# biod/sambamba

Measured on NVIDIA H100. Metric: bam_gb_per_s_depth_base, higher is better.
Workload: dtype u32

## Files before the change

include/bdepth.h:

```cpp
#ifndef BDEPTH_H
#define BDEPTH_H

#include <stddef.h>
#include <stdint.h>

#ifdef __cplusplus
extern "C" {
#endif

typedef struct bdepth bdepth_t;

typedef enum {
    BDEPTH_OK = 0,
    BDEPTH_ERR_IO = -1,
    BDEPTH_ERR_FORMAT = -2,
    BDEPTH_ERR_UNSORTED = -3,
    BDEPTH_ERR_NOINDEX = -4,
    BDEPTH_ERR_CUDA = -5,
    BDEPTH_ERR_NCCL = -6,
    BDEPTH_ERR_ARG = -7,
    BDEPTH_ERR_CALLBACK = -8
} bdepth_status;

typedef struct { uint32_t ref_id, start, end; } bdepth_region;
// ... 34 lines not shown
    uint64_t covered_positions;
    uint64_t long_reads;
    uint64_t chain_fixups;
    uint32_t gpu_launches;
    uint32_t n_batches;
    float ms_h2d, ms_inflate, ms_scan, ms_coverage, ms_reduce, ms_d2h, ms_total_device;
    double host_wall_ms;
    float ms_span_device;
    float ms_exchange;
    uint64_t own_lo, own_hi;
    uint64_t halo_bytes_sent;
    uint64_t mate_pairs;
    uint64_t mate_pair_columns;
    uint64_t mate_groups;
    float ms_mates;
} bdepth_stats;

int  bdepth_device_count(void);
int  bdepth_open(const char* bam_path, int device, bdepth_t** out);
int  bdepth_open_lazy(const char* bam_path, int device, bdepth_t** out);
int  bdepth_open_memory(const void* bam, size_t bam_len, const void* bai, size_t bai_len, int device, bdepth_t** out);
int  bdepth_add_input(bdepth_t* h, const char* bam_path);
void bdepth_close(bdepth_t* h);
const char* bdepth_last_error(const bdepth_t* h);

int         bdepth_n_ref(const bdepth_t* h);
const char* bdepth_ref_name(const bdepth_t* h, int i);
uint32_t    bdepth_ref_length(const bdepth_t* h, int i);
const char* bdepth_header_text(const bdepth_t* h, size_t* len);
int         bdepth_is_coordinate_sorted(const bdepth_t* h);
// ... 54 lines not shown
```

sambamba_b200/_lib.py:

```python
import ctypes as C
import os
import numpy as np

_HERE = os.path.dirname(os.path.abspath(__file__))


def lib_path():
    return os.path.join(_HERE, "_build", "libbdepth.so")


class BDepthError(RuntimeError):
    def __init__(self, code, msg):
        super().__init__(f"bdepth error {code}: {msg}")
        self.code = code
        self.msg = msg


class Region(C.Structure):
    _fields_ = [("ref_id", C.c_uint32), ("start", C.c_uint32), ("end", C.c_uint32)]


class Tile(C.Structure):
    _fields_ = [("ref_id", C.c_int32), ("start", C.c_uint32), ("len", C.c_uint32), ("stride", C.c_uint32),
                ("counts", C.POINTER(C.c_uint32)), ("n_samples", C.c_uint32), ("sample_stride", C.c_uint32)]


class RegionStat(C.Structure):
    _fields_ = [("ref_id", C.c_int32), ("start", C.c_uint32), ("end", C.c_uint32), ("n_reads", C.c_uint32),
                ("n_bases", C.c_uint32), ("cov_ge", C.POINTER(C.c_uint32)), ("sample_id", C.c_int32)]


class Stats(C.Structure):
    _fields_ = [(n, C.c_uint64) for n in ("file_bytes", "n_blocks", "cdata_bytes", "inflated_bytes", "n_records",
                                          "n_records_pass", "n_cigar_ops", "seq_bytes", "positions",
                                          "covered_positions", "long_reads", "chain_fixups")] + \
               [("gpu_launches", C.c_uint32), ("n_batches", C.c_uint32)] + \
               [(n, C.c_float) for n in ("ms_h2d", "ms_inflate", "ms_scan", "ms_coverage", "ms_reduce", "ms_d2h",
                                         "ms_total_device")] + [("host_wall_ms", C.c_double), ("ms_span_device", C.c_float), ("ms_exchange", C.c_float),
                                                                 ("own_lo", C.c_uint64), ("own_hi", C.c_uint64), ("halo_bytes_sent", C.c_uint64),
                                                                 ("mate_pairs", C.c_uint64), ("mate_pair_columns", C.c_uint64), ("mate_groups", C.c_uint64), ("ms_mates", C.c_float)]

    def as_dict(self):
        return {n: getattr(self, n) for n, _ in self._fields_}


FLAGSTAT_FIELDS = ("total", "secondary", "supplementary", "duplicates", "mapped", "paired", "read1", "read2", "proper_pair", "both_mapped",
                   "singletons", "mate_diff_chr", "mate_diff_chr_mapq5")


class FlagStat(C.Structure):
    _fields_ = [(n, C.c_uint64 * 2) for n in FLAGSTAT_FIELDS]

    def as_dict(self):
        return {n: (getattr(self, n)[0], getattr(self, n)[1]) for n in FLAGSTAT_FIELDS}

# ... 359 lines not shown
```

sambamba_b200/csrc/bdepth.cu:

```cuda
#include "launch.cuh"
#include <dlfcn.h>
#include <fcntl.h>
#include <stdarg.h>
#include <stdio.h>
#include <stdlib.h>
#include <sys/mman.h>
#include <sys/stat.h>
#include <unistd.h>
#include <algorithm>
#include <chrono>
#include <map>
#include <string>
#include <vector>

#include "../../include/bdepth.h"
#include "host_bam.hpp"
#include "kernels.cuh"
#include "mates.cuh"
#include "host_filter.hpp"

using namespace bdk;

namespace {

// ... 23 lines not shown
        e = cudaHostGetDevicePointer((void**)&dp, hp, 0);
        if (e == cudaSuccess) cap = n + n / 4;
        used = 0;
        return e;
    }
    uint8_t* take(size_t n) { size_t a = (used + 15) & ~size_t(15); if (a + n > cap) return nullptr; used = a + n; return hp + a; }
    uint8_t* dev(const void* host) const { return dp + ((const uint8_t*)host - hp); }
    void release() { if (hp) cudaFreeHost(hp); hp = nullptr; dp = nullptr; cap = used = 0; }
};
__global__ void k_copy_words(uint32_t* __restrict__ dst, const uint32_t* __restrict__ src, size_t n) {
    for (size_t i = (size_t)blockIdx.x * blockDim.x + threadIdx.x; i < n; i += (size_t)gridDim.x * blockDim.x) dst[i] = src[i];
}

#ifdef BDEPTH_EMULATE_SHIM
constexpr unsigned COUNT_GRID = 4;
#else
constexpr unsigned COUNT_GRID = 2048;
#endif
constexpr size_t CARRY_MAX = 64ull << 20;
constexpr size_t EMIT_CHUNK = 4ull << 20;
constexpr uint32_t SHARD_EXTRA_BLOCKS = 8;
constexpr uint32_t MATE_ZONE_BLOCKS = 64;

enum RunMode { RUN_FULL = 0, RUN_INFLATE_ONLY = 1, RUN_SCAN_ONLY = 2, RUN_INDEX = 3, RUN_FLAGSTAT = 4, RUN_VIEW_COUNT = 5 };
constexpr int RC_RETRY_WINDOW = 1;

struct NcclUid { char b[128]; };
typedef void* NcclComm;
struct NcclApi {
    bool ok = false; std::string err;
    int (*GetUniqueId)(NcclUid*) = nullptr;
    int (*CommInitRank)(NcclComm*, int, NcclUid, int) = nullptr;
// ... 56 lines not shown
    bool k1lz_v12 = false;
    bool k1lz_flat = false;
    int k1h_variant = -1;
    bool k1_onephase = false;
    bool k3_pre = false;
    bool k3_tile = true;
    bool has_fprog = false; FilterProg fprog; DevBuf fprog_d;
    DevBuf m_hash, m_flag, m_flt, m_ctl;
    uint32_t S = 1;
    DevBuf rg_ids, rg_offs, rg_samp;
    DevBuf text[2], text_tiles, text_offs, text_zero, text_samp, present;
    int coll_pending = 0;
    bool want_presence = false;
    uint64_t batch_u = 6ull << 30;
    uint64_t chunk_blocks = 13 * 32 * 16;
    bool shard_ready = false;
    size_t blk_lo = 0, blk_hi = 0; int64_t entry0 = 0; uint64_t limit_abs_u = 0;
    uint64_t zone_lin_lo = UINT64_MAX;
    uint64_t own_lo_abs_u = 0;
    bool sparse_ok = true;
    bool sparse_on = false;
    std::vector<HostBlock> vblocks; std::vector<int32_t> seg_entry ; std::vector<uint32_t> seg_limit ;
    DevBuf anchors_idx, anchors_val, chunk_limit;
    cudaStream_t s_main = nullptr, s_copy = nullptr, s_d2h = nullptr;
    cudaEvent_t ev[32] = {};
    DevBuf comp2[2];
    cudaStream_t s_k1[16] = {};
    std::vector<cudaEvent_t> chunk_ev[2], k1_ev;
    std::vector<size_t> chunk_end[2];
    bool staged = false; uint64_t staged_file_off = 0;
    DevBuf tok, lits, aux, segi, littab;
    DevBuf comp, descs, status, ubuf, chunk_start, entry, exitb, count, slot_base, slots, rec_base, walk_list;
    DevBuf soa_start, soa_span, soa_meta, soa_off, soa_ncl, soa_lseq, long_list, tile_first, tile_lo, counts, ref_len_d, ref_lin0_d, scan_stats, ref_has, ref_has_all, flt_d, lead_list, misc;
    uint64_t cnt_base = 0, win_len = 0;
    void* pinned = nullptr; size_t pinned_cap = 0;
    HostScratch hs;
    std::vector<uint32_t> ref_has_host;
    struct SegSet { bool on = false; uint32_t n = 0; bool has_min = false, has_u = false; uint64_t ext_max = 0; DevBuf s, e, pmax, id, reads, minstart, bases_reads, mbases, ustart, da, dac, db, dthr, dbases, dcov, dscr; } seg;
    struct IndexSet { DevBuf lin, lin_len, lin_base, lin_cap, n_mapped, n_unmapped, carry, ctl, runs, excs; std::vector<uint32_t> base, cap; std::vector<IndexRun> h_runs; std::vector<IndexExc> h_excs; uint64_t n_lin = 0; } ix;
    std::vector<uint8_t> built_bai;
    DevBuf fs; uint64_t fs_host[FS_WORDS + 1] = {};
    ViewSel vsel{}; DevBuf vc, vc_reg, vc_prog; uint64_t vc_host[2] = {};
    std::vector<bdepth*> extra;
    bool accum = false;
    bool force_window = false;
    bdepth_stats st{}; std::string err;
// ... 13 lines not shown
    if (n <= h->pinned_cap) return 0;
    if (h->pinned) cudaFreeHost(h->pinned);
    h->hs.release();
    h->pinned = nullptr; h->pinned_cap = 0;
    CK(cudaMallocHost(&h->pinned, n));
    h->pinned_cap = n;
    return 0;
}

int init_device(bdepth* h) {
    int n = 0; cudaError_t e = cudaGetDeviceCount(&n);
    if (e != cudaSuccess || n <= 0) return fail(h, BDEPTH_ERR_CUDA, "no CUDA device available (%s); libbdepth has no CPU fallback", cudaGetErrorString(e));
    if (h->device < 0 || h->device >= n) return fail(h, BDEPTH_ERR_ARG, "device %d out of range (%d devices)", h->device, n);
    CK(cudaSetDevice(h->device));
    CK(cudaDeviceGetAttribute(&h->n_sm, cudaDevAttrMultiProcessorCount, h->device));
    if (!h->s_main) { CK(cudaStreamCreateWithFlags(&h->s_main, cudaStreamNonBlocking)); CK(cudaStreamCreateWithFlags(&h->s_copy, cudaStreamNonBlocking)); CK(cudaStreamCreateWithFlags(&h->s_d2h, cudaStreamNonBlocking)); for (auto& ks : h->s_k1) CK(cudaStreamCreateWithFlags(&ks, cudaStreamNonBlocking)); for (auto& e2 : h->ev) CK(cudaEventCreate(&e2)); }
    CK(cudaFuncSetAttribute(k1_inflate, cudaFuncAttributeMaxDynamicSharedMemorySize, K1_SMEM));
    CK(cudaFuncSetAttribute(k1_fallback, cudaFuncAttributeMaxDynamicSharedMemorySize, K1_SMEM));
    CK(cudaFuncSetAttribute(k1_huff<false, 4>, cudaFuncAttributePreferredSharedMemoryCarveout, cudaSharedmemCarveoutMaxShared)); CK(cudaFuncSetAttribute(k1_huff<false, 6>, cudaFuncAttributePreferredSharedMemoryCarveout, cudaSharedmemCarveoutMaxShared));
    CK(cudaFuncSetAttribute(k1_huff<true, 5>, cudaFuncAttributePreferredSharedMemoryCarveout, cudaSharedmemCarveoutMaxShared)); CK(cudaFuncSetAttribute(k1_huff<true, 4>, cudaFuncAttributePreferredSharedMemoryCarveout, cudaSharedmemCarveoutMaxShared));
    { const char* e = getenv("BDEPTH_K1H_VARIANT"); h->k1h_variant = e ? atoi(e) : -1; }
    { const char* e = getenv("BDEPTH_K3"); h->k3_tile = !(e && !strcmp(e, "gather")); }
    CK(cudaFuncSetAttribute(k3_tile<false>, cudaFuncAttributeMaxDynamicSharedMemorySize, (int)K3T_SMEM)); CK(cudaFuncSetAttribute(k3_tile<true>, cudaFuncAttributeMaxDynamicSharedMemorySize, (int)K3T_SMEM));
    { const char* e = getenv("BDEPTH_K1LZ"); h->k1lz_flat = e && !strcmp(e, "flat"); h->k1lz_v12 = e && !strcmp(e, "v12"); }
    { const char* e = getenv("BDEPTH_K1_ONEPHASE"); h->k1_onephase = e && atoi(e) == 1; }
    { const char* e = getenv("BDEPTH_K3_PREFETCH"); h->k3_pre = !e || atoi(e) != 0; }
    return 0;
}

int inflate_blocks_to_host(bdepth* h, size_t b0, size_t b1, std::vector<uint8_t>& out) {
    size_t nb = b1 - b0; if (!nb) { out.clear(); return 0; }
// ... 335 lines not shown
__global__ void k_scatter_i64(int64_t* __restrict__ dst, const uint32_t* __restrict__ idx, const int64_t* __restrict__ val, uint32_t n) {
    uint32_t i = blockIdx.x * blockDim.x + threadIdx.x; if (i < n) dst[idx[i]] = val[i];
}

struct RunOut {
    uint8_t* inflate_dst = nullptr; uint64_t inflate_cap = 0; uint64_t inflate_len = 0;
    uint64_t scan_cap = 0; uint64_t scan_n = 0;
    int32_t* ref_id = nullptr; int32_t* pos = nullptr; uint32_t* span = nullptr; uint16_t* flag = nullptr; uint8_t* mapq = nullptr; uint16_t* n_cigar = nullptr; uint64_t* rec_off = nullptr;
};

__global__ void k_fill_u32(uint32_t* p, uint32_t v, uint64_t n) { uint64_t i = (uint64_t)blockIdx.x * blockDim.x + threadIdx.x; if (i < n) p[i] = v; }

int run_pipeline_body(bdepth* h, RunMode mode, RunOut* ro, Emitter* em);
int run_pipeline(bdepth* h, RunMode mode, RunOut* ro, Emitter* em = nullptr) {
    const int rc = run_pipeline_body(h, mode, ro, em);
    if (rc && rc != RC_RETRY_WINDOW) abort_collectives(h);
    return rc;
}
int run_pipeline_body(bdepth* h, RunMode mode, RunOut* ro, Emitter* em) {
    h->coll_pending = 0;
    int rc = init_device(h); if (rc) return rc;
    auto t_host0 = std::chrono::steady_clock::now();
    bdepth_stats& st = h->st; uint32_t launches0 = 0;
    st = bdepth_stats{}; st.gpu_launches = launches0;
    const bool sparse = (mode == RUN_FULL || mode == RUN_VIEW_COUNT) && plan_sparse(h);
    h->coll_pending = (mode == RUN_FULL && h->world > 1 && h->comm) ? (sparse ? 2 : 1) : (mode == RUN_FLAGSTAT && h->world > 1 && h->comm) ? 3 : (mode == RUN_VIEW_COUNT && h->world > 1 && h->comm) ? (sparse ? 2 : 4) : 0;
    if (!sparse) { rc = prepare_shard(h); if (rc) return rc; }
    const bool fix = mode == RUN_FULL && h->fix_mates;
    bool flt_uploaded = false;
    if (fix && h->world > 1 && !h->comm) return fail(h, BDEPTH_ERR_ARG, "fix-mate-overlaps on several ranks needs the boundary exchange (bdepth_set_shard with a NCCL id)");
// ... 172 lines not shown
            const HostBlock& hb = B[b + i];
            uint64_t dev_off = h->staged ? hb.coff - h->staged_file_off : dco[batch_no & 1][i];
            d[i] = BlockDesc{dev_off + hb.cdata_off, hb.uoff - batch_u0, hb.csize, hb.isize, tok_words};
            tok_words += tok_cap_of(hb.isize);
            if (b + i >= new_b) { csum += hb.csize; st.file_bytes += hb.bsize; }
        }
        st.cdata_bytes += csum;
        CK(h->descs.ensure(nb * sizeof(BlockDesc))); CK(h->status.ensure(nb * sizeof(int))); CK(h->ubuf.ensure(CARRY_MAX + ub + 256));
        if (!h->k1_onephase) { CK(h->tok.ensure(tok_words * 4 + 64)); CK(h->lits.ensure(ub + 16 * nb + 64)); CK(h->aux.ensure(nb * sizeof(BlockAux))); CK(h->segi.ensure(nb * MAX_SEG * 4)); CK(h->littab.ensure(nb * (size_t)MAX_SEG * 256)); }
        CK(hs.ensure(nb * (sizeof(BlockDesc) + 192) + 16384)); hs.used = 0;
        UP(h->descs.p, d.data(), nb * sizeof(BlockDesc));
        uint8_t* u0 = h->ubuf.as<uint8_t>() + CARRY_MAX;
        CK(cudaEventRecord(e1, sm));
        struct Sub { size_t s0, s1; int ev_lo, ev_hi; };
        std::vector<Sub> subs;
        auto launch_k1 = [&](cudaStream_t ks, size_t c0, uint32_t n) -> int {
            const BlockDesc* dd = h->descs.as<BlockDesc>() + (c0 - b); int* stp = h->status.as<int>() + (c0 - b);
            if (h->k1_onephase) {
                BD_LAUNCH((n + 32 * K1_WARPS - 1) / (32 * K1_WARPS), 32 * K1_WARPS, K1_SMEM, ks, k1_inflate)(d_comp, dd, n, u0, stp);
                CK(cudaGetLastError()); st.gpu_launches++;
                return 0;
            }
            BlockAux* ax = h->aux.as<BlockAux>() + (c0 - b); uint32_t* sgi = h->segi.as<uint32_t>() + (c0 - b) * MAX_SEG; uint8_t* ltb = h->littab.as<uint8_t>() + (c0 - b) * (size_t)MAX_SEG * 256;
            const unsigned hg = (n + 32 * K1H_WARPS - 1) / (32 * K1H_WARPS); const uint32_t blk0 = (uint32_t)(c0 - b);
#define K1H(LIMS, MINB) BD_LAUNCH(hg, 32 * K1H_WARPS, k1h_smem<LIMS>(), ks, k1_huff<LIMS, MINB>)(d_comp, dd, n, blk0, stp, h->tok.as<uint32_t>(), h->lits.as<uint8_t>(), ax, sgi, ltb)
            const int variant = h->k1h_variant >= 0 ? h->k1h_variant : (n > (uint32_t)h->n_sm * 16u * 32u ? 2 : 0);
            switch (variant) { case 1: K1H(false, 6); break; case 2: K1H(true, 5); break; case 3: K1H(true, 4); break; default: K1H(false, 4); }
#undef K1H
            if (h->k1lz_flat) BD_LAUNCH((n + K1L_WARPS - 1) / K1L_WARPS, 32 * K1L_WARPS, 0, ks, k1_lz_flat)(dd, n, blk0, u0, stp, h->tok.as<uint32_t>(), h->lits.as<uint8_t>(), ax, sgi, ltb);
            else if (h->k1lz_v12) BD_LAUNCH((n + K1L_WARPS - 1) / K1L_WARPS, 32 * K1L_WARPS, 0, ks, k1_lz<false>)(dd, n, blk0, u0, stp, h->tok.as<uint32_t>(), h->lits.as<uint8_t>(), ax, sgi, ltb);
            else BD_LAUNCH((n + K1L_WARPS - 1) / K1L_WARPS, 32 * K1L_WARPS, 0, ks, k1_lz<true>)(dd, n, blk0, u0, stp, h->tok.as<uint32_t>(), h->lits.as<uint8_t>(), ax, sgi, ltb);
            BD_LAUNCH((n + 32 * K1_WARPS - 1) / (32 * K1_WARPS), 32 * K1_WARPS, K1_SMEM, ks, k1_fallback)(d_comp, dd, n, u0, stp);
            CK(cudaGetLastError()); st.gpu_launches += 3;
            return 0;
        };
        if (h->staged) {
            { int rck = launch_k1(sm, b, (uint32_t)nb); if (rck) return rck; }
            subs.push_back(Sub{b, b1, 0, -1});
        } else {
            int slot = (int)(batch_no & 1); size_t c0 = b;
            for (size_t j = 0; j < h->chunk_end[slot].size(); j++) {
                size_t c1 = h->chunk_end[slot][j]; cudaStream_t ks = h->s_k1[j & 15];
                CK(cudaStreamWaitEvent(ks, e1, 0)); CK(cudaStreamWaitEvent(ks, h->chunk_ev[slot][j], 0));
                uint32_t n = (uint32_t)(c1 - c0);
                { int rck = launch_k1(ks, c0, n); if (rck) return rck; }
                if (h->k1_ev.size() <= j) { cudaEvent_t ne; CK(cudaEventCreateWithFlags(&ne, cudaEventDisableTiming)); h->k1_ev.push_back(ne); }
                CK(cudaEventRecord(h->k1_ev[j], ks));
                if ((mode == RUN_FULL || mode == RUN_INDEX || mode == RUN_FLAGSTAT || mode == RUN_VIEW_COUNT) && !fix) subs.push_back(Sub{c0, c1, (int)j, (int)j}); else { if (subs.empty()) subs.push_back(Sub{b, b1, 0, (int)j}); subs[0].ev_hi = (int)j; }
                c0 = c1;
            }
        }
        if (!h->staged && !fix && b1 < blk_hi) { int rcp = issue_h2d(batch_no + 1, b1, batch_end(b1)); if (rcp) return rcp; }
        const size_t mb = b, mb1 = b1; const uint64_t m_u0abs = batch_u0; uint8_t* const m_u0 = u0; const bool m_last = last_batch;
        for (size_t sbi = 0; sbi < subs.size(); sbi++) {
        const size_t b = subs[sbi].s0, b1 = subs[sbi].s1, nb = b1 - b;
        const uint64_t batch_u0 = B[b].uoff, ub = B[b1 - 1].uoff + B[b1 - 1].isize - batch_u0;
        uint8_t* const u0 = m_u0 + (batch_u0 - m_u0abs);
        const bool last_sub = sbi + 1 == subs.size(), last_batch = m_last && last_sub;
        for (int j = subs[sbi].ev_lo; j <= subs[sbi].ev_hi; j++) CK(cudaStreamWaitEvent(sm, h->k1_ev[j], 0));
        CK(cudaEventRecord(e2, sm));
        if (!h->staged && last_sub) CK(cudaEventRecord(h->ev[16 + (batch_no & 1)], sm));
        DOWN(stt, int, h->status.as<int>() + (b - mb), nb * sizeof(int));
        if (mode == RUN_INFLATE_ONLY) {
            CK(cudaStreamSynchronize(sm));
            for (size_t i = 0; i < nb; i++) if (stt[i]) return fail(h, BDEPTH_ERR_FORMAT, "DEFLATE error %d in BGZF block at offset %llu", stt[i], (unsigned long long)B[b + i].coff);
            if (ro && ro->inflate_dst) {
                if (ro->inflate_len + ub > ro->inflate_cap) return fail(h, BDEPTH_ERR_ARG, "inflate buffer too small");
                CK(cudaMemcpy(ro->inflate_dst + ro->inflate_len, u0, ub, cudaMemcpyDeviceToHost));
            }
            if (ro) ro->inflate_len += ub;
            float t; CK(cudaEventElapsedTime(&t, e1, e2)); ms_k1 += t;
            continue;
        }
        const bool seg0 = sparse && h->seg_entry[b] >= 0;
        if (seg0) carry_len = 0;
        std::vector<int64_t> cstart(nb + 1); std::vector<uint32_t> sbase(nb + 1);
        { uint64_t acc = 0; for (size_t i = 0; i < nb; i++) { cstart[i] = (int64_t)(B[b + i].uoff - batch_u0); sbase[i] = (uint32_t)acc; uint64_t sz = B[b + i].isize + (i == 0 ? carry_len : 0); acc += sz / 36 + 2; } cstart[nb] = (int64_t)ub; sbase[nb] = (uint32_t)acc; cstart[0] = -(int64_t)carry_len;
          if (acc > 0xFFFFFFFFull) return fail(h, BDEPTH_ERR_ARG, "batch too large"); }
        const uint64_t n_slots = sbase[nb];
        CK(h->chunk_start.ensure((nb + 1) * 8)); CK(h->slot_base.ensure((nb + 1) * 4)); CK(h->entry.ensure(nb * 8)); CK(h->exitb.ensure(nb * 8)); CK(h->count.ensure(nb * 4)); CK(h->rec_base.ensure((nb + 1) * 4)); CK(h->slots.ensure(n_slots * 2 + 64)); CK(h->walk_list.ensure(64));
// ... 17 lines not shown
            CK(h->chunk_limit.ensure(nb * 8)); UP(h->chunk_limit.p, lim.data(), nb * 8); d_limit = h->chunk_limit.as<int64_t>();
            if (!ai.empty()) {
                CK(h->anchors_idx.ensure(ai.size() * 4)); CK(h->anchors_val.ensure(av.size() * 8));
                UP(h->anchors_idx.p, ai.data(), ai.size() * 4); UP(h->anchors_val.p, av.data(), av.size() * 8);
                BD_LAUNCH((unsigned)((ai.size() + 255) / 256), 256, 0, sm, k_scatter_i64)(h->entry.as<int64_t>(), h->anchors_idx.as<uint32_t>(), h->anchors_val.as<int64_t>(), (uint32_t)ai.size());
                CK(cudaGetLastError()); st.gpu_launches++;
            }
        }
        ScanParams spw = sp;
        BD_LAUNCH((unsigned)((nb + 127) / 128), 128, 0, sm, k2_walk)(spw, h->chunk_start.as<int64_t>(), (uint32_t)nb, h->entry.as<int64_t>(), h->slot_base.as<uint32_t>(), h->slots.as<uint16_t>(), h->count.as<uint32_t>(), h->exitb.as<int64_t>(), (int*)h->misc.p, nullptr, 0, d_limit);
        CK(cudaGetLastError()); st.gpu_launches++;
        DOWN(ent, int64_t, h->entry.p, nb * 8); DOWN(ext, int64_t, h->exitb.p, nb * 8); DOWN(cnt, uint32_t, h->count.p, nb * 4);
        DOWN(werr, int, h->misc.p, 4);
        CK(cudaStreamSynchronize(sm));
        int walk_err = *werr;
        for (size_t i = 0; i < nb; i++) if (stt[i]) return fail(h, BDEPTH_ERR_FORMAT, "DEFLATE error %d in BGZF block at offset %llu", stt[i], (unsigned long long)B[b + i].coff);
        int64_t cur = anchor; int64_t tail = (int64_t)ub;
        for (size_t i = 0; i < nb; i++) {
            if (sparse && i && h->seg_entry[b + i] >= 0) cur = cstart[i] + h->seg_entry[b + i];
            int64_t true_e = (cur < cstart[i + 1]) ? cur : ENTRY_NONE;
            if (true_e != ENTRY_NONE && true_e < cstart[i]) return fail(h, BDEPTH_ERR_FORMAT, "internal: record chain went backwards");
            if (ent[i] != true_e) {
                st.chain_fixups++;
                uint32_t ci = (uint32_t)i;
                UP((int64_t*)h->entry.p + i, &true_e, 8);
                UP(h->walk_list.p, &ci, 4);
                BD_LAUNCH(1, 32, 0, sm, k2_walk)(spw, h->chunk_start.as<int64_t>(), (uint32_t)nb, h->entry.as<int64_t>(), h->slot_base.as<uint32_t>(), h->slots.as<uint16_t>(), h->count.as<uint32_t>(), h->exitb.as<int64_t>(), (int*)h->misc.p, h->walk_list.as<uint32_t>(), 1, d_limit);
                CK(cudaGetLastError()); st.gpu_launches++;
                DOWN(fx_ext, int64_t, (int64_t*)h->exitb.p + i, 8); DOWN(fx_cnt, uint32_t, (uint32_t*)h->count.p + i, 4); DOWN(fx_err, int, h->misc.p, 4);
                CK(cudaStreamSynchronize(sm));
                ext[i] = *fx_ext; cnt[i] = *fx_cnt; walk_err = *fx_err;
// ... 232 lines not shown
            BD_LAUNCH((unsigned)((R + 255) / 256), 256, 0, sm, k_view_count)(soa, u0, (uint32_t)R, own_from, h->vsel, h->vc.as<unsigned long long>());
            CK(cudaGetLastError()); st.gpu_launches++;
            CK(cudaEventRecord(h->ev[23], sm));
        }
        const bool zone_mode = h->world > 1 && h->comm && !fix && !sparse;
        if (em && zone_mode && h->rank > 0 && shard_min != UINT64_MAX) em->lo_clip = shard_min;
        if (em && mode == RUN_FULL && (h->world == 1 || (zone_mode && (h->rank == 0 || shard_min != UINT64_MAX))) && !fix && !last_batch && ss.n_pass) { int rce = em->advance(ss.max_start / TILE_POS * TILE_POS, e4); if (rce) return rce; }
        uint64_t new_carry = (uint64_t)((int64_t)ub - tail);
        if (last_batch && last_sub && !sparse && !limited && b1 == B.size() && new_carry >= 4) return fail(h, BDEPTH_ERR_FORMAT, "truncated BAM record at the end of the file (not enough data in stream)");
        if (!last_batch && last_sub && new_carry && !fix) {
            if (new_carry > CARRY_MAX) return fail(h, BDEPTH_ERR_FORMAT, "BAM record larger than %zu bytes", CARRY_MAX);
            CK(cudaMemcpyAsync(m_u0 - new_carry, u0 + tail, new_carry, cudaMemcpyDeviceToDevice, sm));
        }
        CK(cudaStreamSynchronize(sm));
        if ((mode == RUN_FLAGSTAT || mode == RUN_VIEW_COUNT) && R) { float t; CK(cudaEventElapsedTime(&t, h->ev[22], h->ev[23])); ms_census += t; }
        { float t; if (!h->staged && last_sub) { CK(cudaEventElapsedTime(&t, h->ev[18 + (batch_no & 1)], h->ev[14 + (batch_no & 1)])); ms_h2d += t; } if (last_sub) { CK(cudaEventElapsedTime(&t, e1, e2)); ms_k1 += t; } CK(cudaEventElapsedTime(&t, e2, e3)); ms_k2 += t; CK(cudaEventElapsedTime(&t, e3, e4)); ms_k3 += t; }
        carry_len = (last_batch || fix) ? 0 : new_carry; first_batch = false;
        hs.used = 0;
        }
        if (sparse_bad) break;
        }
        b = b1; batch_no++;
    }
    if (sparse && h->world > 1) {
        if (h->comm) {
            uint32_t flag = sparse_bad ? 1u : 0u;
            CK(cudaMemcpyAsync(h->misc.p, &flag, 4, cudaMemcpyHostToDevice, sm));
            NK(nccl().AllReduce(h->misc.p, h->misc.p, 1, NCCL_UINT32, NCCL_SUM, h->comm, sm));
            h->coll_pending = mode == RUN_VIEW_COUNT ? 4 : 1;
            CK(cudaMemcpyAsync(&flag, h->misc.p, 4, cudaMemcpyDeviceToHost, sm)); CK(cudaStreamSynchronize(sm));
            if (flag >= SPARSE_PEER_FAILED) { h->coll_pending = 0; return fail(h, BDEPTH_ERR_NCCL, "another rank of the run stopped with an error (its own message says why): no result"); }
// ... 269 lines not shown
long bdepth_plan_region_chunks(const char* bam_path, const bdepth_region* regions, size_t n, uint64_t* out_pairs, size_t cap) {
    if (!bam_path || (n && !regions)) return fail(nullptr, BDEPTH_ERR_ARG, "bad argument");
    BaiIndex bai;
    { std::string p1 = std::string(bam_path) + ".bai"; FILE* f = fopen(p1.c_str(), "rb"); if (!f) return fail(nullptr, BDEPTH_ERR_NOINDEX, "no index %s", p1.c_str());
      fseek(f, 0, SEEK_END); long nb = ftell(f); fseek(f, 0, SEEK_SET); std::vector<uint8_t> buf(nb); if (fread(buf.data(), 1, nb, f) != (size_t)nb) { fclose(f); return fail(nullptr, BDEPTH_ERR_IO, "read error"); } fclose(f);
      if (!parse_bai(buf.data(), buf.size(), bai)) return fail(nullptr, BDEPTH_ERR_FORMAT, "bad BAI"); }
    std::vector<HostRegion> rg;
    for (size_t i = 0; i < n; i++) if (regions[i].start < regions[i].end) rg.push_back(HostRegion{regions[i].ref_id, regions[i].start, regions[i].end});
    std::sort(rg.begin(), rg.end(), [](const HostRegion& a, const HostRegion& b) { return a.ref != b.ref ? a.ref < b.ref : a.start < b.start; });
    std::vector<BaiChunk> cs = region_chunks(bai, rg);
    for (size_t i = 0; i < cs.size() && i < cap; i++) { out_pairs[2 * i] = cs[i].beg; out_pairs[2 * i + 1] = cs[i].end; }
    return (long)cs.size();
}
int bdepth_set_tuning(bdepth_t* h, uint64_t batch_inflated_bytes, uint64_t chunk_blocks) {
    if (batch_inflated_bytes) h->batch_u = std::max<uint64_t>(batch_inflated_bytes, 1 << 16);
    if (chunk_blocks) h->chunk_blocks = chunk_blocks;
    h->staged = false;
    return 0;
}

int bdepth_stage(bdepth_t* h) {
    int rc = init_device(h); if (rc) return rc;
    rc = prepare_shard(h); if (rc) return rc;
    if (h->blk_lo >= h->blk_hi) { h->staged = false; return 0; }
    const auto& B = h->blocks;
    uint64_t f0 = B[h->blk_lo].coff & ~3ull, f1 = B[h->blk_hi - 1].coff + B[h->blk_hi - 1].bsize;
    CK(h->comp.ensure(f1 - f0 + 256));
    CK(cudaMemcpyAsync(h->comp.p, h->file + f0, f1 - f0, cudaMemcpyHostToDevice, h->s_main));
    CK(cudaMemsetAsync((uint8_t*)h->comp.p + (f1 - f0), 0, 128, h->s_main));
    CK(cudaStreamSynchronize(h->s_main));
    h->staged = true; h->staged_file_off = f0;
// ... 480 lines not shown
```

sambamba_b200/csrc/inflate2_core.cuh:

```cuda
#pragma once
#include "inflate_core.cuh"

namespace bdk {

constexpr int INF_FALLBACK = 100;
constexpr int MAX_SEG = 8;
constexpr uint32_t SEG_RAW = 1u << 31;
constexpr uint32_t TOK_NOMATCH = 1u << 31;
constexpr uint32_t LIT_RUN_MAX = 252;

constexpr int H_LL = 0;
constexpr int H_NL = 32;
constexpr int H_DD = 40;
constexpr int H_DS = 48;
constexpr int H_WORDS = 56;
constexpr int H_SMEM_BYTES_PER_WARP = H_WORDS * 128 + 32 * 64;

struct SmemTab2 {
    uint32_t* base;
    uint32_t* lim;
    uint32_t fifo_sa;
    BD_HD uint32_t ldw(int w) const { return base[w * 32]; }
    BD_HD void stw(int w, uint32_t v) const { base[w * 32] = v; }
    BD_HD void st_lim(int which, const uint32_t* pk) const { for (int i = 0; i < 8; i++) lim[(which * 2 + (i >> 2)) * 128 + (i & 3)] = pk[i]; }
// ... 370 lines not shown
```

sambamba_b200/csrc/kernels.cuh:

```cuda
#pragma once
#include "launch.cuh"
#include <stdint.h>
#include "inflate_core.cuh"
#include "inflate2_core.cuh"
#include "filter.cuh"

namespace bdk {

constexpr int TILE_POS = 1024;
constexpr uint32_t SPAN_SHORT = 1024;
constexpr int N_PLANES = 7;
constexpr int64_t ENTRY_NONE = (int64_t)0x8080808080808080ull;
constexpr int ENTRY_NONE_BYTE = 0x80;

struct BlockDesc {
    uint64_t coff;
    uint64_t uoff;
    uint32_t csize;
    uint32_t isize;
    uint64_t tok_off;
};
BD_HD uint32_t tok_cap_of(uint32_t isize) { return isize / 4u + 16u; }
struct BlockAux { uint32_t n_tok, n_seg, n_lit, pad; };
BD_HD uint64_t lit_off_of(uint64_t uoff, uint64_t block_index) { return (uoff & ~15ull) + 16ull * block_index; }
// ... 9 lines not shown
    const bool active = b < n_blocks;
    BlockDesc d = active ? blocks[b] : BlockDesc{0, 0, 0, 0, 0};
    uint32_t* wbase = smem + warp * (SMEM_BYTES_PER_WARP / 4);
    SmemTab tab{wbase + lane, (uint32_t)__cvta_generic_to_shared(wbase + T_WORDS * 32) + lane * 16, (uint32_t)__cvta_generic_to_shared(wbase + T_FAR * 32 + lane)};
    ByteOut out{u};
    int rc = inflate_block(tab, comp, d.coff, d.csize, out, d.uoff, d.isize, scratch, active);
    if (active) status[b] = rc;
}


constexpr int K1H_WARPS = 4;
template <bool LIMS> constexpr int k1h_smem() { return K1H_WARPS * (H_SMEM_BYTES_PER_WARP + (LIMS ? H_LIM_BYTES_PER_WARP : 0)); }
template <bool LIMS, int MINB>
__global__ void __launch_bounds__(K1H_WARPS * 32, MINB) k1_huff(const uint32_t* __restrict__ comp, const BlockDesc* __restrict__ blocks, uint32_t n_blocks, uint32_t blk0,
                                                                int* __restrict__ status, uint32_t* __restrict__ tok, uint8_t* __restrict__ lits, BlockAux* __restrict__ aux,
                                                                uint32_t* __restrict__ seg_info, uint8_t* __restrict__ lit_tab) {
    BD_DYN_SMEM(uint32_t, smem);
    uint32_t lane = threadIdx.x & 31, warp = threadIdx.x >> 5;
    uint32_t b = (blockIdx.x * K1H_WARPS + warp) * 32u + lane;
    uint32_t scratch[96];
    const bool active = b < n_blocks;
    BlockDesc d = active ? blocks[b] : BlockDesc{0, 0, 0, 0, 0};
    constexpr int PER_WARP = (H_SMEM_BYTES_PER_WARP + (LIMS ? H_LIM_BYTES_PER_WARP : 0)) / 4;
    uint32_t* wbase = smem + warp * PER_WARP;
    uint32_t* limb = wbase + H_WORDS * 32 + (32 * RING_BYTES_PER_LANE) / 4;
    SmemTab2 tab{wbase + lane, limb + lane * 4, (uint32_t)__cvta_generic_to_shared(wbase + H_WORDS * 32) + lane * 16};
    HuffOut ho{tok + d.tok_off, tok_cap_of(d.isize), lits + lit_off_of(d.uoff, (uint64_t)blk0 + b), lit_tab + (size_t)b * (MAX_SEG * 256), seg_info + (size_t)b * MAX_SEG};
    uint32_t n_tok = 0, n_seg = 0, n_lit = 0;
    int rc = huff_phase<SmemTab2, LIMS>(tab, comp, d.coff, d.csize, d.isize, scratch, ho, n_tok, n_seg, n_lit, active);
    if (active) { status[b] = rc; aux[b] = BlockAux{n_tok, n_seg, n_lit, 0u}; }
}

__device__ __forceinline__ uint32_t ld_u32_any(const uint8_t* p) {
    uintptr_t a = reinterpret_cast<uintptr_t>(p); const uint32_t* w = reinterpret_cast<const uint32_t*>(a & ~uintptr_t(3));
    return __funnelshift_r(w[0], w[1], (uint32_t)(a & 3) * 8);
}
constexpr int K1L_WARPS = 8;
#ifndef BDEPTH_EMULATE_SHIM
__device__ __forceinline__ uint32_t warp_max_u32(uint32_t v) { return __reduce_max_sync(0xFFFFFFFFu, v); }
#else
static inline uint32_t warp_max_u32(uint32_t v) { return ~__reduce_min_sync(0xFFFFFFFFu, ~v); }
static inline bool emu_k1lz_warp() { static const bool on = getenv("BDEPTH_EMU_K1LZ_WARP") && atoi(getenv("BDEPTH_EMU_K1LZ_WARP")) == 1; return on; }
#endif
template <bool COMPACT>
__global__ void __launch_bounds__(K1L_WARPS * 32, 6) k1_lz(const BlockDesc* __restrict__ blocks, uint32_t n_blocks, uint32_t blk0, uint8_t* __restrict__ u, int* __restrict__ status,
// ... 176 lines not shown
                        s = ms - dd + (dd <= k ? k % dd : k);
                    }
                    if (!done) v = ub[s];
                }
                ub[base + o] = (uint8_t)v;
            }
        }
        base += tot; lbase += totl;
        __syncwarp();
    }
    if (!err && (base != d.isize || lbase != ax.n_lit)) err = INF_ERR_SHORT;
    if (err && lane == 0) status[b] = err;
}

__global__ void __launch_bounds__(K1_WARPS * 32, 1) k1_fallback(const uint32_t* __restrict__ comp, const BlockDesc* __restrict__ blocks,
                                                                uint32_t n_blocks, uint8_t* __restrict__ u, int* __restrict__ status) {
    BD_DYN_SMEM(uint32_t, smem);
    uint32_t lane = threadIdx.x & 31, warp = threadIdx.x >> 5;
    uint32_t b = (blockIdx.x * K1_WARPS + warp) * 32u + lane;
    uint32_t scratch[96];
    const bool active = b < n_blocks && status[b] == INF_FALLBACK;
#ifndef BDEPTH_EMULATE_SHIM
    if (!__any_sync(0xFFFFFFFFu, active)) return;
#endif
    BlockDesc d = active ? blocks[b] : BlockDesc{0, 0, 0, 0, 0};
    uint32_t* wbase = smem + warp * (SMEM_BYTES_PER_WARP / 4);
    SmemTab tab{wbase + lane, (uint32_t)__cvta_generic_to_shared(wbase + T_WORDS * 32) + lane * 16, (uint32_t)__cvta_generic_to_shared(wbase + T_FAR * 32 + lane)};
    ByteOut out{u};
    int rc = inflate_block(tab, comp, d.coff, d.csize, out, d.uoff, d.isize, scratch, active);
    if (active) status[b] = rc;
}

__device__ __forceinline__ uint32_t ldu32(const uint8_t* p) {
    uintptr_t a = reinterpret_cast<uintptr_t>(p);
    const uint32_t* w = reinterpret_cast<const uint32_t*>(a & ~uintptr_t(3));
    uint32_t lo = __ldg(w), hi = __ldg(w + 1);
    return __funnelshift_r(lo, hi, (uint32_t)(a & 3) * 8);
}
__device__ __forceinline__ uint32_t ldu16(const uint8_t* p) { return ldu32(p) & 0xFFFFu; }

struct ScanParams {
    const uint8_t* u;
    int64_t u_begin;
    int64_t u_end;
    int n_ref;
// ... 1027 lines not shown
```

Baseline: 46.35.

## Split staged inflate into one Huffman pass, compacted fallback, and chunked LZ

When the BAM is staged on the device, the Huffman phase now runs once over the whole batch. Blocks that need the slow path are recorded in a compacted list through an atomic counter, so the fallback kernel launches only over those blocks instead of scanning every block. The LZ phase is then issued in chunks with per-chunk events so downstream scan and coverage work can start on early chunks. The main stream is also given the highest stream priority. This adds a host sync to read the fallback count and a new INF_REDONE status code that the error checks must accept.

```diff
diff --git a/include/bdepth.h b/include/bdepth.h
--- a/include/bdepth.h
+++ b/include/bdepth.h
@@ -72,6 +72,9 @@
     uint64_t mate_pair_columns;
     uint64_t mate_groups;
     float ms_mates;
+    float ms_inflate_huff;
+    uint32_t k1_fallback_blocks;
+    uint64_t k1_chunk_blocks;
 } bdepth_stats;
 
 int  bdepth_device_count(void);
diff --git a/sambamba_b200/_lib.py b/sambamba_b200/_lib.py
--- a/sambamba_b200/_lib.py
+++ b/sambamba_b200/_lib.py
@@ -38,7 +38,8 @@
                [(n, C.c_float) for n in ("ms_h2d", "ms_inflate", "ms_scan", "ms_coverage", "ms_reduce", "ms_d2h",
                                          "ms_total_device")] + [("host_wall_ms", C.c_double), ("ms_span_device", C.c_float), ("ms_exchange", C.c_float),
                                                                  ("own_lo", C.c_uint64), ("own_hi", C.c_uint64), ("halo_bytes_sent", C.c_uint64),
-                                                                 ("mate_pairs", C.c_uint64), ("mate_pair_columns", C.c_uint64), ("mate_groups", C.c_uint64), ("ms_mates", C.c_float)]
+                                                                 ("mate_pairs", C.c_uint64), ("mate_pair_columns", C.c_uint64), ("mate_groups", C.c_uint64), ("ms_mates", C.c_float),
+                                                                 ("ms_inflate_huff", C.c_float), ("k1_fallback_blocks", C.c_uint32), ("k1_chunk_blocks", C.c_uint64)]
 
     def as_dict(self):
         return {n: getattr(self, n) for n, _ in self._fields_}
diff --git a/sambamba_b200/csrc/bdepth.cu b/sambamba_b200/csrc/bdepth.cu
--- a/sambamba_b200/csrc/bdepth.cu
+++ b/sambamba_b200/csrc/bdepth.cu
@@ -61,8 +61,13 @@
 
 #ifdef BDEPTH_EMULATE_SHIM
 constexpr unsigned COUNT_GRID = 4;
+static inline cudaError_t create_high_priority_stream(cudaStream_t* s) { return cudaStreamCreateWithFlags(s, cudaStreamNonBlocking); }
 #else
 constexpr unsigned COUNT_GRID = 2048;
+static inline cudaError_t create_high_priority_stream(cudaStream_t* s) {
+    int least = 0, greatest = 0; cudaError_t e = cudaDeviceGetStreamPriorityRange(&least, &greatest); if (e != cudaSuccess) return e;
+    return cudaStreamCreateWithPriority(s, cudaStreamNonBlocking, greatest);
+}
 #endif
 constexpr size_t CARRY_MAX = 64ull << 20;
 constexpr size_t EMIT_CHUNK = 4ull << 20;
@@ -149,6 +154,7 @@
     bool want_presence = false;
     uint64_t batch_u = 6ull << 30;
     uint64_t chunk_blocks = 13 * 32 * 16;
+    bool chunk_blocks_set = false;
     bool shard_ready = false;
     size_t blk_lo = 0, blk_hi = 0; int64_t entry0 = 0; uint64_t limit_abs_u = 0;
     uint64_t zone_lin_lo = UINT64_MAX;
@@ -165,6 +171,7 @@
     std::vector<size_t> chunk_end[2];
     bool staged = false; uint64_t staged_file_off = 0;
     DevBuf tok, lits, aux, segi, littab;
+    DevBuf fb;
     DevBuf comp, descs, status, ubuf, chunk_start, entry, exitb, count, slot_base, slots, rec_base, walk_list;
     DevBuf soa_start, soa_span, soa_meta, soa_off, soa_ncl, soa_lseq, long_list, tile_first, tile_lo, counts, ref_len_d, ref_lin0_d, scan_stats, ref_has, ref_has_all, flt_d, lead_list, misc;
     uint64_t cnt_base = 0, win_len = 0;
@@ -208,7 +215,7 @@
     if (h->device < 0 || h->device >= n) return fail(h, BDEPTH_ERR_ARG, "device %d out of range (%d devices)", h->device, n);
     CK(cudaSetDevice(h->device));
     CK(cudaDeviceGetAttribute(&h->n_sm, cudaDevAttrMultiProcessorCount, h->device));
-    if (!h->s_main) { CK(cudaStreamCreateWithFlags(&h->s_main, cudaStreamNonBlocking)); CK(cudaStreamCreateWithFlags(&h->s_copy, cudaStreamNonBlocking)); CK(cudaStreamCreateWithFlags(&h->s_d2h, cudaStreamNonBlocking)); for (auto& ks : h->s_k1) CK(cudaStreamCreateWithFlags(&ks, cudaStreamNonBlocking)); for (auto& e2 : h->ev) CK(cudaEventCreate(&e2)); }
+    if (!h->s_main) { CK(create_high_priority_stream(&h->s_main)); CK(cudaStreamCreateWithFlags(&h->s_copy, cudaStreamNonBlocking)); CK(cudaStreamCreateWithFlags(&h->s_d2h, cudaStreamNonBlocking)); for (auto& ks : h->s_k1) CK(cudaStreamCreateWithFlags(&ks, cudaStreamNonBlocking)); for (auto& e2 : h->ev) CK(cudaEventCreate(&e2)); }
     CK(cudaFuncSetAttribute(k1_inflate, cudaFuncAttributeMaxDynamicSharedMemorySize, K1_SMEM));
     CK(cudaFuncSetAttribute(k1_fallback, cudaFuncAttributeMaxDynamicSharedMemorySize, K1_SMEM));
     CK(cudaFuncSetAttribute(k1_huff<false, 4>, cudaFuncAttributePreferredSharedMemoryCarveout, cudaSharedmemCarveoutMaxShared)); CK(cudaFuncSetAttribute(k1_huff<false, 6>, cudaFuncAttributePreferredSharedMemoryCarveout, cudaSharedmemCarveoutMaxShared));
@@ -574,6 +581,7 @@
 int run_pipeline_body(bdepth* h, RunMode mode, RunOut* ro, Emitter* em);
 int run_pipeline(bdepth* h, RunMode mode, RunOut* ro, Emitter* em = nullptr) {
     const int rc = run_pipeline_body(h, mode, ro, em);
+    if (rc) for (auto& ks : h->s_k1) if (ks) cudaStreamSynchronize(ks);
     if (rc && rc != RC_RETRY_WINDOW) abort_collectives(h);
     return rc;
 }
@@ -776,6 +784,27 @@
         CK(cudaEventRecord(e1, sm));
         struct Sub { size_t s0, s1; int ev_lo, ev_hi; };
         std::vector<Sub> subs;
+        auto launch_huff = [&](cudaStream_t ks, size_t c0, uint32_t n, uint32_t* fb) -> int {
+            const BlockDesc* dd = h->descs.as<BlockDesc>() + (c0 - b); int* stp = h->status.as<int>() + (c0 - b);
+            BlockAux* ax = h->aux.as<BlockAux>() + (c0 - b); uint32_t* sgi = h->segi.as<uint32_t>() + (c0 - b) * MAX_SEG; uint8_t* ltb = h->littab.as<uint8_t>() + (c0 - b) * (size_t)MAX_SEG * 256;
+            const unsigned hg = (n + 32 * K1H_WARPS - 1) / (32 * K1H_WARPS); const uint32_t blk0 = (uint32_t)(c0 - b);
+#define K1H(LIMS, MINB) BD_LAUNCH(hg, 32 * K1H_WARPS, k1h_smem<LIMS>(), ks, k1_huff<LIMS, MINB>)(d_comp, dd, n, blk0, stp, h->tok.as<uint32_t>(), h->lits.as<uint8_t>(), ax, sgi, ltb, fb)
+            const int variant = h->k1h_variant >= 0 ? h->k1h_variant : (n > (uint32_t)h->n_sm * 16u * 32u ? 2 : 0);
+            switch (variant) { case 1: K1H(false, 6); break; case 2: K1H(true, 5); break; case 3: K1H(true, 4); break; default: K1H(false, 4); }
+#undef K1H
+            CK(cudaGetLastError()); st.gpu_launches++;
+            return 0;
+        };
+        auto launch_lz = [&](cudaStream_t ks, size_t c0, uint32_t n) -> int {
+            const BlockDesc* dd = h->descs.as<BlockDesc>() + (c0 - b); int* stp = h->status.as<int>() + (c0 - b);
+            BlockAux* ax = h->aux.as<BlockAux>() + (c0 - b); uint32_t* sgi = h->segi.as<uint32_t>() + (c0 - b) * MAX_SEG; uint8_t* ltb = h->littab.as<uint8_t>() + (c0 - b) * (size_t)MAX_SEG * 256;
+            const uint32_t blk0 = (uint32_t)(c0 - b);
+            if (h->k1lz_flat) BD_LAUNCH((n + K1L_WARPS - 1) / K1L_WARPS, 32 * K1L_WARPS, 0, ks, k1_lz_flat)(dd, n, blk0, u0, stp, h->tok.as<uint32_t>(), h->lits.as<uint8_t>(), ax, sgi, ltb);
+            else if (h->k1lz_v12) BD_LAUNCH((n + K1L_WARPS - 1) / K1L_WARPS, 32 * K1L_WARPS, 0, ks, k1_lz<false>)(dd, n, blk0, u0, stp, h->tok.as<uint32_t>(), h->lits.as<uint8_t>(), ax, sgi, ltb);
+            else BD_LAUNCH((n + K1L_WARPS - 1) / K1L_WARPS, 32 * K1L_WARPS, 0, ks, k1_lz<true>)(dd, n, blk0, u0, stp, h->tok.as<uint32_t>(), h->lits.as<uint8_t>(), ax, sgi, ltb);
+            CK(cudaGetLastError()); st.gpu_launches++;
+            return 0;
+        };
         auto launch_k1 = [&](cudaStream_t ks, size_t c0, uint32_t n) -> int {
             const BlockDesc* dd = h->descs.as<BlockDesc>() + (c0 - b); int* stp = h->status.as<int>() + (c0 - b);
             if (h->k1_onephase) {
@@ -783,20 +812,40 @@
                 CK(cudaGetLastError()); st.gpu_launches++;
                 return 0;
             }
-            BlockAux* ax = h->aux.as<BlockAux>() + (c0 - b); uint32_t* sgi = h->segi.as<uint32_t>() + (c0 - b) * MAX_SEG; uint8_t* ltb = h->littab.as<uint8_t>() + (c0 - b) * (size_t)MAX_SEG * 256;
-            const unsigned hg = (n + 32 * K1H_WARPS - 1) / (32 * K1H_WARPS); const uint32_t blk0 = (uint32_t)(c0 - b);
-#define K1H(LIMS, MINB) BD_LAUNCH(hg, 32 * K1H_WARPS, k1h_smem<LIMS>(), ks, k1_huff<LIMS, MINB>)(d_comp, dd, n, blk0, stp, h->tok.as<uint32_t>(), h->lits.as<uint8_t>(), ax, sgi, ltb)
-            const int variant = h->k1h_variant >= 0 ? h->k1h_variant : (n > (uint32_t)h->n_sm * 16u * 32u ? 2 : 0);
-            switch (variant) { case 1: K1H(false, 6); break; case 2: K1H(true, 5); break; case 3: K1H(true, 4); break; default: K1H(false, 4); }
-#undef K1H
-            if (h->k1lz_flat) BD_LAUNCH((n + K1L_WARPS - 1) / K1L_WARPS, 32 * K1L_WARPS, 0, ks, k1_lz_flat)(dd, n, blk0, u0, stp, h->tok.as<uint32_t>(), h->lits.as<uint8_t>(), ax, sgi, ltb);
-            else if (h->k1lz_v12) BD_LAUNCH((n + K1L_WARPS - 1) / K1L_WARPS, 32 * K1L_WARPS, 0, ks, k1_lz<false>)(dd, n, blk0, u0, stp, h->tok.as<uint32_t>(), h->lits.as<uint8_t>(), ax, sgi, ltb);
-            else BD_LAUNCH((n + K1L_WARPS - 1) / K1L_WARPS, 32 * K1L_WARPS, 0, ks, k1_lz<true>)(dd, n, blk0, u0, stp, h->tok.as<uint32_t>(), h->lits.as<uint8_t>(), ax, sgi, ltb);
-            BD_LAUNCH((n + 32 * K1_WARPS - 1) / (32 * K1_WARPS), 32 * K1_WARPS, K1_SMEM, ks, k1_fallback)(d_comp, dd, n, u0, stp);
-            CK(cudaGetLastError()); st.gpu_launches += 3;
+            { int rc1 = launch_huff(ks, c0, n, nullptr); if (rc1) return rc1; }
+            { int rc2 = launch_lz(ks, c0, n); if (rc2) return rc2; }
+            BD_LAUNCH((n + 32 * K1_WARPS - 1) / (32 * K1_WARPS), 32 * K1_WARPS, K1_SMEM, ks, k1_fallback)(d_comp, dd, n, u0, stp, nullptr);
+            CK(cudaGetLastError()); st.gpu_launches++;
             return 0;
         };
-        if (h->staged) {
+        const bool sub_batched = (mode == RUN_FULL || mode == RUN_INDEX || mode == RUN_FLAGSTAT || mode == RUN_VIEW_COUNT) && !fix;
+        const bool staged_split = h->staged && !h->k1_onephase;
+        if (staged_split) {
+            cudaStream_t ks = h->s_k1[0];
+            CK(cudaStreamWaitEvent(ks, e1, 0));
+            CK(h->fb.ensure((nb + 1) * 4)); CK(cudaMemsetAsync(h->fb.p, 0, 4, ks));
+            { int rck = launch_huff(ks, b, (uint32_t)nb, h->fb.as<uint32_t>()); if (rck) return rck; }
+            CK(cudaEventRecord(h->ev[24], ks));
+            uint32_t n_fb = 0;
+            CK(cudaMemcpyAsync(&n_fb, h->fb.p, 4, cudaMemcpyDeviceToHost, ks)); CK(cudaStreamSynchronize(ks));
+            if (n_fb) {
+                BD_LAUNCH((n_fb + 32 * K1_WARPS - 1) / (32 * K1_WARPS), 32 * K1_WARPS, K1_SMEM, ks, k1_fallback)(d_comp, h->descs.as<BlockDesc>(), n_fb, u0, h->status.as<int>(), h->fb.as<uint32_t>() + 1);
+                CK(cudaGetLastError()); st.gpu_launches++;
+            }
+            st.k1_fallback_blocks += n_fb;
+            const size_t step = h->chunk_blocks_set ? h->chunk_blocks : nb;
+            st.k1_chunk_blocks = step;
+            size_t c0 = b;
+            for (size_t j = 0; c0 < b1; j++) {
+                const size_t c1 = std::min(b1, c0 + step);
+                { int rck = launch_lz(ks, c0, (uint32_t)(c1 - c0)); if (rck) return rck; }
+                if (h->k1_ev.size() <= j) { cudaEvent_t ne; CK(cudaEventCreateWithFlags(&ne, cudaEventDisableTiming)); h->k1_ev.push_back(ne); }
+                CK(cudaEventRecord(h->k1_ev[j], ks));
+                if (sub_batched) subs.push_back(Sub{c0, c1, (int)j, (int)j}); else { if (subs.empty()) subs.push_back(Sub{b, b1, 0, (int)j}); subs[0].ev_hi = (int)j; }
+                c0 = c1;
+            }
+            CK(cudaEventRecord(h->ev[25], ks));
+        } else if (h->staged) {
             { int rck = launch_k1(sm, b, (uint32_t)nb); if (rck) return rck; }
             subs.push_back(Sub{b, b1, 0, -1});
         } else {
@@ -808,7 +857,7 @@
                 { int rck = launch_k1(ks, c0, n); if (rck) return rck; }
                 if (h->k1_ev.size() <= j) { cudaEvent_t ne; CK(cudaEventCreateWithFlags(&ne, cudaEventDisableTiming)); h->k1_ev.push_back(ne); }
                 CK(cudaEventRecord(h->k1_ev[j], ks));
-                if ((mode == RUN_FULL || mode == RUN_INDEX || mode == RUN_FLAGSTAT || mode == RUN_VIEW_COUNT) && !fix) subs.push_back(Sub{c0, c1, (int)j, (int)j}); else { if (subs.empty()) subs.push_back(Sub{b, b1, 0, (int)j}); subs[0].ev_hi = (int)j; }
+                if (sub_batched) subs.push_back(Sub{c0, c1, (int)j, (int)j}); else { if (subs.empty()) subs.push_back(Sub{b, b1, 0, (int)j}); subs[0].ev_hi = (int)j; }
                 c0 = c1;
             }
         }
@@ -825,7 +874,7 @@
         DOWN(stt, int, h->status.as<int>() + (b - mb), nb * sizeof(int));
         if (mode == RUN_INFLATE_ONLY) {
             CK(cudaStreamSynchronize(sm));
-            for (size_t i = 0; i < nb; i++) if (stt[i]) return fail(h, BDEPTH_ERR_FORMAT, "DEFLATE error %d in BGZF block at offset %llu", stt[i], (unsigned long long)B[b + i].coff);
+            for (size_t i = 0; i < nb; i++) if (stt[i] && stt[i] != INF_REDONE) return fail(h, BDEPTH_ERR_FORMAT, "DEFLATE error %d in BGZF block at offset %llu", stt[i], (unsigned long long)B[b + i].coff);
             if (ro && ro->inflate_dst) {
                 if (ro->inflate_len + ub > ro->inflate_cap) return fail(h, BDEPTH_ERR_ARG, "inflate buffer too small");
                 CK(cudaMemcpy(ro->inflate_dst + ro->inflate_len, u0, ub, cudaMemcpyDeviceToHost));
@@ -873,7 +922,7 @@
         DOWN(werr, int, h->misc.p, 4);
         CK(cudaStreamSynchronize(sm));
         int walk_err = *werr;
-        for (size_t i = 0; i < nb; i++) if (stt[i]) return fail(h, BDEPTH_ERR_FORMAT, "DEFLATE error %d in BGZF block at offset %llu", stt[i], (unsigned long long)B[b + i].coff);
+        for (size_t i = 0; i < nb; i++) if (stt[i] && stt[i] != INF_REDONE) return fail(h, BDEPTH_ERR_FORMAT, "DEFLATE error %d in BGZF block at offset %llu", stt[i], (unsigned long long)B[b + i].coff);
         int64_t cur = anchor; int64_t tail = (int64_t)ub;
         for (size_t i = 0; i < nb; i++) {
             if (sparse && i && h->seg_entry[b + i] >= 0) cur = cstart[i] + h->seg_entry[b + i];
@@ -1136,7 +1185,7 @@
         }
         CK(cudaStreamSynchronize(sm));
         if ((mode == RUN_FLAGSTAT || mode == RUN_VIEW_COUNT) && R) { float t; CK(cudaEventElapsedTime(&t, h->ev[22], h->ev[23])); ms_census += t; }
-        { float t; if (!h->staged && last_sub) { CK(cudaEventElapsedTime(&t, h->ev[18 + (batch_no & 1)], h->ev[14 + (batch_no & 1)])); ms_h2d += t; } if (last_sub) { CK(cudaEventElapsedTime(&t, e1, e2)); ms_k1 += t; } CK(cudaEventElapsedTime(&t, e2, e3)); ms_k2 += t; CK(cudaEventElapsedTime(&t, e3, e4)); ms_k3 += t; }
+        { float t; if (!h->staged && last_sub) { CK(cudaEventElapsedTime(&t, h->ev[18 + (batch_no & 1)], h->ev[14 + (batch_no & 1)])); ms_h2d += t; } if (last_sub) { CK(cudaEventElapsedTime(&t, e1, staged_split ? h->ev[25] : e2)); ms_k1 += t; } if (last_sub && staged_split) { CK(cudaEventElapsedTime(&t, e1, h->ev[24])); st.ms_inflate_huff += t; } CK(cudaEventElapsedTime(&t, e2, e3)); ms_k2 += t; CK(cudaEventElapsedTime(&t, e3, e4)); ms_k3 += t; }
         carry_len = (last_batch || fix) ? 0 : new_carry; first_batch = false;
         hs.used = 0;
         }
@@ -1436,7 +1485,7 @@
 }
 int bdepth_set_tuning(bdepth_t* h, uint64_t batch_inflated_bytes, uint64_t chunk_blocks) {
     if (batch_inflated_bytes) h->batch_u = std::max<uint64_t>(batch_inflated_bytes, 1 << 16);
-    if (chunk_blocks) h->chunk_blocks = chunk_blocks;
+    if (chunk_blocks) { h->chunk_blocks = chunk_blocks; h->chunk_blocks_set = true; }
     h->staged = false;
     return 0;
 }
diff --git a/sambamba_b200/csrc/inflate2_core.cuh b/sambamba_b200/csrc/inflate2_core.cuh
--- a/sambamba_b200/csrc/inflate2_core.cuh
+++ b/sambamba_b200/csrc/inflate2_core.cuh
@@ -4,6 +4,7 @@
 namespace bdk {
 
 constexpr int INF_FALLBACK = 100;
+constexpr int INF_REDONE = 101;
 constexpr int MAX_SEG = 8;
 constexpr uint32_t SEG_RAW = 1u << 31;
 constexpr uint32_t TOK_NOMATCH = 1u << 31;
diff --git a/sambamba_b200/csrc/kernels.cuh b/sambamba_b200/csrc/kernels.cuh
--- a/sambamba_b200/csrc/kernels.cuh
+++ b/sambamba_b200/csrc/kernels.cuh
@@ -47,7 +47,7 @@
 template <bool LIMS, int MINB>
 __global__ void __launch_bounds__(K1H_WARPS * 32, MINB) k1_huff(const uint32_t* __restrict__ comp, const BlockDesc* __restrict__ blocks, uint32_t n_blocks, uint32_t blk0,
                                                                 int* __restrict__ status, uint32_t* __restrict__ tok, uint8_t* __restrict__ lits, BlockAux* __restrict__ aux,
-                                                                uint32_t* __restrict__ seg_info, uint8_t* __restrict__ lit_tab) {
+                                                                uint32_t* __restrict__ seg_info, uint8_t* __restrict__ lit_tab, uint32_t* __restrict__ fb) {
     BD_DYN_SMEM(uint32_t, smem);
     uint32_t lane = threadIdx.x & 31, warp = threadIdx.x >> 5;
     uint32_t b = (blockIdx.x * K1H_WARPS + warp) * 32u + lane;
@@ -62,6 +62,7 @@
     uint32_t n_tok = 0, n_seg = 0, n_lit = 0;
     int rc = huff_phase<SmemTab2, LIMS>(tab, comp, d.coff, d.csize, d.isize, scratch, ho, n_tok, n_seg, n_lit, active);
     if (active) { status[b] = rc; aux[b] = BlockAux{n_tok, n_seg, n_lit, 0u}; }
+    if (active && rc == INF_FALLBACK && fb) fb[1 + atomicAdd(fb, 1u)] = blk0 + b;
 }
 
 __device__ __forceinline__ uint32_t ld_u32_any(const uint8_t* p) {
@@ -268,12 +269,13 @@
 }
 
 __global__ void __launch_bounds__(K1_WARPS * 32, 1) k1_fallback(const uint32_t* __restrict__ comp, const BlockDesc* __restrict__ blocks,
-                                                                uint32_t n_blocks, uint8_t* __restrict__ u, int* __restrict__ status) {
+                                                                uint32_t n_blocks, uint8_t* __restrict__ u, int* __restrict__ status, const uint32_t* __restrict__ list) {
     BD_DYN_SMEM(uint32_t, smem);
     uint32_t lane = threadIdx.x & 31, warp = threadIdx.x >> 5;
-    uint32_t b = (blockIdx.x * K1_WARPS + warp) * 32u + lane;
+    const uint32_t i = (blockIdx.x * K1_WARPS + warp) * 32u + lane;
+    const uint32_t b = (list && i < n_blocks) ? list[i] : i;
     uint32_t scratch[96];
-    const bool active = b < n_blocks && status[b] == INF_FALLBACK;
+    const bool active = i < n_blocks && status[b] == INF_FALLBACK;
 #ifndef BDEPTH_EMULATE_SHIM
     if (!__any_sync(0xFFFFFFFFu, active)) return;
 #endif
@@ -282,7 +284,7 @@
     SmemTab tab{wbase + lane, (uint32_t)__cvta_generic_to_shared(wbase + T_WORDS * 32) + lane * 16, (uint32_t)__cvta_generic_to_shared(wbase + T_FAR * 32 + lane)};
     ByteOut out{u};
     int rc = inflate_block(tab, comp, d.coff, d.csize, out, d.uoff, d.isize, scratch, active);
-    if (active) status[b] = rc;
+    if (active) status[b] = (list && rc == INF_OK) ? INF_REDONE : rc;
 }
 
 __device__ __forceinline__ uint32_t ldu32(const uint8_t* p) {
```

Result: no change. 46.18, median of 6 (-0.4%).
